# at-cg/PHI

Hardware: AMD Instinct MI355X
Metric: read Gbases/s scored (49-hap MHC graph stand-in synMHC-49); reads resident in HBM, parsing and H2D excluded (higher is better)
Workload: dtype u64

## Files before the change

phi_amd/build.py:

```python
import os
import subprocess
import sys

ROOT = os.path.dirname(os.path.dirname(os.path.abspath(__file__)))
CSRC = os.path.join(ROOT, "phi_amd", "csrc")
HIPCC = os.environ.get("HIPCC", "/opt/rocm/bin/hipcc")
ARCH = "gfx950"

HIP_SOURCES = ["sketch.hip", "sketch_pooled.hip", "sketch_win_fixed.hip", "table.hip", "anchors.hip", "contexts.hip", "dp.hip", "dp_events.hip", "dp_blocks.hip", "phi_abi.hip", "dev_mem.hip", "read_batches.hip", "text_stream.hip", "text_park.hip", "set_graph.hip", "phi_solve.hip", "solve_dev.hip", "phi_comm.hip", "phi_ipc.hip", "reads_text.hip", "walk_text.hip", "edit.hip", "edit_path.hip", "inflate.hip", "gfa_text.hip", "chop.hip", "vcf.hip", "ladder.hip", "panel.hip", "panel_score.hip", "scan.hip", "bam.hip", "calls.hip", "deflate.hip"]
HIP_HEADERS = ["phi_dev.h", "phi_kernels.h", "phi_ctx.h", "phi_dp_flags.h", "phi_host_par.h", "phi_wave.h", "dp_dev.h", "dp_steps.h", "solve_host.h", "reads_host.h", "bam_header.h", "deflate_codes.h", "sketch_dev.h", "sketch_phases.inc", "sketch_minima.inc", "sketch_rounds.inc", "sketch_rounds_kmer.inc", "edit_band.inc", os.path.join("host", "panel_choose.h"), os.path.join("..", "..", "include", "phi_amd.h")]


def _run(cmd, cwd=None):
    print("+", " ".join(cmd), flush=True)
    subprocess.check_call(cmd, cwd=cwd)


def _stale(target, deps):
    if not os.path.exists(target):
        return True
    t = os.path.getmtime(target)
    return any(os.path.getmtime(d) > t for d in deps if os.path.exists(d))


EXTRA_FLAGS = {"sketch_pooled.hip": ["-mllvm", "-disable-machine-licm"]}


def build_device(force=False):
    objdir = os.path.join(ROOT, "build", "obj")
    os.makedirs(objdir, exist_ok=True)
    hdrs = [os.path.join(CSRC, h) for h in HIP_HEADERS]
    objs = []
    for src in HIP_SOURCES:
        s = os.path.join(CSRC, src)
        o = os.path.join(objdir, src.replace(".hip", ".o"))
        if force or _stale(o, [s] + hdrs):
            _run([HIPCC, f"--offload-arch={ARCH}", "-O3", "-std=c++17", "-fPIC", "-Wall", "-Wno-unused-function"]
                 + EXTRA_FLAGS.get(src, []) + ["-c", s, "-o", o])
        objs.append(o)
    lib = os.path.join(ROOT, "phi_amd", "libphi_amd.so")
    if force or _stale(lib, objs):
        tmp = f"{lib}.{os.getpid()}.tmp"
        _run([HIPCC, f"--offload-arch={ARCH}", "-shared", "-fPIC", "-o", tmp] + objs + ["-ldl"])
        os.replace(tmp, lib)
    return lib


def build_host(force=False):
    hostdir = os.path.join(CSRC, "host")
    if not os.path.isdir(hostdir):
        return None
    _run(["make", "-C", hostdir] + (["-B"] if force else []))
    return os.path.join(ROOT, "phi_amd", "libphi_host.so")


def build_all(force=False):
    build_device(force)
    build_host(force)


if __name__ == "__main__":
    build_all(force="--force" in sys.argv)
```

phi_amd/csrc/dp_events.hip:

```cpp
#include <hip/hip_runtime.h>
#include "phi_kernels.h"
#include "dp_dev.h"

#define CHK PHI_DP_CHUNK
#define RING PHI_DP_RING
enum { DP_SEQ = 0, DP_ROW = 1, DP_PATH = 2 };

__global__ void __launch_bounds__(256) phi_event_flags_kernel(const int32_t *__restrict__ walk_vtx, int64_t n_entries,
                                                              const int32_t *__restrict__ cvtx, uint8_t *__restrict__ flags)
{
    for (int64_t e = (int64_t)blockIdx.x * blockDim.x + threadIdx.x; e < n_entries; e += (int64_t)gridDim.x * blockDim.x)
        flags[e] = cvtx[walk_vtx[e]] >= 0;
}

__global__ void phi_event_off_kernel(const phi_ent_t *__restrict__ ev_e, int64_t n_ev, const int64_t *__restrict__ walk_off,
                                     int32_t n_walks, int64_t *__restrict__ ev_off)
{
    const int h = blockIdx.x * blockDim.x + threadIdx.x;
    if (h > n_walks) return;
    const int64_t key = walk_off[h];
    int64_t lo = 0, hi = n_ev;
    while (lo < hi) {
        const int64_t mid = (lo + hi) >> 1;
        if ((int64_t)ev_e[mid] < key) lo = mid + 1; else hi = mid;
// ... 167 lines not shown
    const int h = threadIdx.x;
    const bool has_walk = h < A.n_walks;
    const int64_t eb = has_walk ? A.walk_off[h] : 0;
    const int64_t ee = has_walk ? A.walk_off[h + 1] : 0;
    const int32_t sb = MODE == DP_PATH ? (int32_t)blockIdx.x : 0;
    const int32_t kbeg = MODE == DP_PATH ? A.blk_lo[sb] : 0, kend = MODE == DP_PATH ? A.blk_lo[sb + 1] : A.n_k;
    const int64_t vb = !has_walk ? 0 : MODE == DP_PATH ? (int64_t)A.blk_ev[(int64_t)sb * A.lane_stride + h] : A.ev_off[h];
    const int64_t ve = has_walk ? A.ev_off[h + 1] : 0;
    int64_t vi = vb;
    int64_t wl = vb;
    const uint4 *evg = reinterpret_cast<const uint4 *>(A.ev);

    uint4 wtmp[P][3];
    int64_t whi = vb;
    auto issue = [&]() {
        whi = min(ve, vi + D);
#pragma unroll
        for (int j = 0; j < P; j++) {
            const int64_t x = (ve > vb) ? min(wl + j, ve - 1) : 0;
            wtmp[j][0] = evg[x * 3 + 0]; wtmp[j][1] = evg[x * 3 + 1]; wtmp[j][2] = evg[x * 3 + 2];
        }
    };
    auto land = [&]() {
#pragma unroll
        for (int j = 0; j < P; j++) {
            const int64_t x = wl + j;
            if (x < whi) {
                const int sl = (int)(x & (D - 1));
                s_ev[sl][0][h] = wtmp[j][0]; s_ev[sl][1][h] = wtmp[j][1]; s_ev[sl][2][h] = wtmp[j][2];
            }
        }
        wl = max(wl, min(whi, wl + P));
    };
    if (A.n_ev > 0) { issue(); land(); issue(); land(); }
    uint4 cA = make_uint4(0xFFFFFFFFu, 0, 0, 0);
    if (vi < ve) cA = s_ev[vi & (D - 1)][0][h];

    int32_t qh = 0, qt = 0;
    int32_t M = NEGK, sL = 0, Emax = NEG;
    if (MODE == DP_PATH) { sL = -1; if (has_walk) M = A.blk_S[(int64_t)sb * A.lane_stride + h]; }

    const int32_t n_steps = kend - kbeg;
    const int n_chunks = (n_steps + CHK - 1) / CHK;
    auto stage = [&](int c) {
        const int b = c & 1;
        const int32_t s0 = kbeg + c * CHK;
        const int32_t ns = min(CHK, kend - s0);
        const int4 *src = reinterpret_cast<const int4 *>(A.k_rec + (int64_t)s0 * 8);
        int4 *dst = &s_rec[b][0][0];
        for (int i = h; i < ns * 2; i += NT) dst[i] = src[i];
    };
    stage(0);
    __syncthreads();

    for (int c = 0; c < n_chunks; c++) {
        const int b = c & 1;
        if (c + 1 < n_chunks) stage(c + 1);
        const int32_t s0 = kbeg + c * CHK;
        const int32_t ns = min(CHK, kend - s0);
        int4 ra = s_rec[b][0][0], rb = s_rec[b][0][1];
        for (int i = 0; i < ns; i++) {
            const int inx = min(i + 1, CHK - 1);
            const int4 na = s_rec[b][inx][0], nb = s_rec[b][inx][1];
            if ((c | i) && (i & (P - 1)) == 0) issue();
            if ((c | i) && (i & (P - 1)) == P / 2) {
                land();
                if (vi < ve) cA = s_ev[vi & (D - 1)][0][h];
            }
            const int32_t k = s0 + i;
            const int32_t flags = ra.x;
            const bool active = (int32_t)(cA.x & 0x7FFFFFFFu) == k;

            int32_t E = NEG, Eh = -1, Esrc = -1;
            if (flags & PHI_DP_NEED_ENTRY) {
                dp_eval_entry<RNG, true>(ra, rb, k, s_top, A.k_in_packed, reinterpret_cast<const int4 *>(A.tops), A.cost, E, Eh, Esrc);
                if (h == 0) { A.ent_src[k] = Esrc; A.ent_h[k] = Eh; }
            }

            int32_t dmax = NEG;
            int32_t oidx = 255;
            if (active) {
                const int64_t e = (int64_t)cA.y;
                const bool ovf = (cA.x >> 31) != 0;
                const int32_t t = (int32_t)(e - eb);
                const int32_t End = (int32_t)cA.z, SB = (int32_t)cA.w;
                const int sl = (int)(vi & (D - 1));
                const uint8_t *gb = reinterpret_cast<const uint8_t *>(&s_ev[sl][1][h]);
                oidx = reinterpret_cast<const uint8_t *>(&s_ev[sl][2][h])[15];
                while (qh != qt && t - s_qs[qh & (QD - 1)][h] >= 31) {
                    const int32_t key = s_qK[qh & (QD - 1)][h];
                    if (key > M) { M = key; sL = s_qs[qh & (QD - 1)][h]; }
                    qh++;
                }
                int32_t newE = NEG;
                if (t == 0) { newE = 0; qh = qt = 0; M = NEGK; Emax = NEG; }
                else if ((flags & PHI_DP_NEED_ENTRY) && Eh >= 0) newE = E;
                if (newE > Emax) {
                    Emax = newE;
                    const int32_t key = newE - SB;
                    while (qh != qt && s_qK[(qt - 1) & (QD - 1)][h] < key) qt--;
                    if (qt - qh >= q_limit) { atomicOr(A.err, PHI_KERR_DP_QUEUE); qt--; }
                    s_qs[qt & (QD - 1)][h] = t; s_qE[qt & (QD - 1)][h] = newE; s_qK[qt & (QD - 1)][h] = key;
                    qt++;
                }
                if ((flags & PHI_DP_NEED_TOPS) || e == ee - 1) {
                    int32_t best = M > NEGK / 2 ? M + End : NEG, bs = sL;
                    for (int32_t j = qh; j != qt; j++) {
                        const int32_t s = s_qs[j & (QD - 1)][h];
                        const int a = t - s;
                        int32_t inside;
                        if (!ovf) inside = a < 16 ? gb[a] : reinterpret_cast<const uint8_t *>(&s_ev[sl][2][h])[a - 16];
                        else inside = ev_count_inside(A, eb + s, e);
                        const int32_t val = s_qE[j & (QD - 1)][h] + inside;
                        if (val > best) { best = val; bs = s; }
                    }
                    if (best > NEG / 2) { dmax = best; A.dmax[e] = best; A.bstart[e] = bs; }
                    else { A.dmax[e] = NEG; A.bstart[e] = 0; }
                }
                vi++;
                cA = make_uint4(0xFFFFFFFFu, 0, 0, 0);
                if (vi < ve) cA = s_ev[vi & (D - 1)][0][h];
            }

            if (flags & PHI_DP_NEED_TOPS) {
                const bool leaving = active && oidx != 255 && dmax > NEG / 2;
                const DpTops t = dp_tops_waves<NW>(leaving, dmax, oidx, s_red, s_oidx);
                if (h == 0) {
                    const int4 q = pack_tops(t);
                    s_top[k & (RNG - 1)] = q;
                    reinterpret_cast<int4 *>(A.tops)[k] = q;
                }
                __syncthreads();
            }
            ra = na; rb = nb;
        }
        __threadfence_block();
        __syncthreads();
    }
    if (MODE == DP_PATH) {
        int32_t best = M > NEGK / 2 ? M : NEGK, bs = sL;
        for (int32_t j = qh; j != qt; j++) {
            const int32_t key = s_qK[j & (QD - 1)][h];
            if (key > best) { best = key; bs = s_qs[j & (QD - 1)][h]; }
        }
        A.blk_keys_out[(int64_t)sb * A.lane_stride + h] = (has_walk && vb < ve) ? best : NEGK;
        A.blk_carry[(int64_t)sb * A.lane_stride + h] = bs;
    }
}


template <int NPW, int MODE, int P, int RINGT, int QD, int CK = CHK>
__global__ void __launch_bounds__(64 * (1 + NPW)) phi_dp_events_pc_kernel(PhiDpEventArgs A)
{
    constexpr int D = 2 * P;
    constexpr int PER_CHUNK = CK / P;
    static_assert(P % NPW == 0 && CK % P == 0, "ring geometry");
    __shared__ int4 s_rec[2 * CK][2];
    __shared__ int4 s_top[RINGT];
    __shared__ int2 s_ent[2 * P];
    __shared__ uint4 s_ev[D][3][64];
    __shared__ int4 s_res[D][64];
    __shared__ int32_t s_qs[QD][64], s_qE[QD][64], s_qK[QD][64];
    __shared__ int32_t s_vi[2][64];

    const int wave = threadIdx.x >> 6, h = threadIdx.x & 63;
    const bool cls = MODE == DP_ROW && A.lane_walk != nullptr;
    const unsigned n_rows = cls ? 65u : (unsigned)(A.n_walks + 1);
    int32_t sb = 0, row_j = -1;
    if (MODE == DP_ROW) { sb = (int32_t)(blockIdx.x / n_rows); row_j = (int32_t)(blockIdx.x % n_rows); }
    if (MODE == DP_PATH) sb = (int32_t)blockIdx.x;
    const bool start_row = MODE == DP_ROW && row_j == (int32_t)n_rows - 1;
    int32_t w = h;
    bool has_walk = h < A.n_walks;
    if (cls) { w = A.lane_walk[(int64_t)sb * 64 + h]; has_walk = w >= 0; if (!has_walk) w = 0; }
    const int32_t k0 = MODE == DP_SEQ ? 0 : A.blk_lo[sb];
    const int32_t k1 = MODE == DP_SEQ ? A.n_k : A.blk_lo[sb + 1];
    const int32_t n_steps = k1 - k0;
    const phi_ent_t eb = has_walk ? (phi_ent_t)A.walk_off[w] : 0;
    const phi_ent_t e_last = has_walk ? (phi_ent_t)(A.walk_off[w + 1] - 1) : 0xFFFFFFFFu;
    const int32_t v0 = has_walk ? (int32_t)A.ev_off[w] : 0;
    const int32_t ve = has_walk ? (int32_t)A.ev_off[w + 1] : 0;
    const int32_t vb = MODE == DP_SEQ ? v0 : (has_walk ? A.blk_ev[(int64_t)sb * A.lane_stride + w] : 0);
    const int n_per = (n_steps + P - 1) / P;
    if (MODE == DP_ROW && !start_row) {
        const int32_t wj = cls ? A.lane_walk[(int64_t)sb * 64 + row_j] : row_j;
        if (wj < 0) return;
        const int32_t jb = A.blk_ev[(int64_t)sb * A.lane_stride + wj];
        if (jb <= (int32_t)A.ev_off[wj] || jb >= (int32_t)A.ev_off[wj + 1]) {
            if (wave == 0) {
                A.row_out[(int64_t)blockIdx.x * 64 + h] = NEGK;
                if (h == 0) { A.rowend_out[blockIdx.x] = NEG; if (A.rownew_out) A.rownew_out[blockIdx.x] = NEGK; if (A.rowdiag_out) A.rowdiag_out[(int64_t)sb * 64 + row_j] = NEGK; }
            }
            return;
        }
    }

    if (wave > 0) {
        const int pw = wave - 1;
        const uint4 *evg = reinterpret_cast<const uint4 *>(A.ev);
        auto stage = [&](int c) {
            const int32_t s0 = k0 + c * CK;
            const int32_t ns = min(CK, k1 - s0);
            const int4 *src = reinterpret_cast<const int4 *>(A.k_rec + (int64_t)s0 * 8);
            int4 *dst = &s_rec[(c & 1) * CK][0];
            for (int i = pw * 64 + h; i < ns * 2; i += 64 * NPW) dst[i] = src[i];
        };
        stage(0);
#pragma unroll
        for (int n = 0; n < D / NPW; n++) {
            const int32_t x = vb + pw + n * NPW;
            if (x < ve) {
                const uint4 a = evg[(int64_t)x * 3 + 0], g0 = evg[(int64_t)x * 3 + 1], g1 = evg[(int64_t)x * 3 + 2];
                s_ev[x & (D - 1)][0][h] = a; s_ev[x & (D - 1)][1][h] = g0; s_ev[x & (D - 1)][2][h] = g1;
            }
        }
        int32_t wl = min(ve, vb + D);
        int32_t vprev = vb;
        __syncthreads();
        for (int p = 0;; p++) {
            const int32_t vi = has_walk ? s_vi[p & 1][h] : 0;
            if (MODE != DP_ROW) {
#pragma unroll
                for (int n = 0; n < P / NPW; n++) {
                    const int32_t x = vprev + pw + n * NPW;
                    if (x < vi) {
                        const int4 r = s_res[x & (D - 1)][h];
                        A.dmax[(phi_ent_t)r.z] = r.x; A.bstart[(phi_ent_t)r.z] = r.y;
                    }
                }
                if (pw == 0 && p > 0 && h < P) {
                    const int32_t r = (p - 1) * P + h;
                    if (r < n_steps) {
                        const int32_t k = k0 + r;
                        reinterpret_cast<int4 *>(A.tops)[k] = s_top[k & (RINGT - 1)];
                        const int2 en = s_ent[r & (2 * P - 1)];
                        A.ent_src[k] = en.x; A.ent_h[k] = en.y;
                    }
                }
            }
            if (p == n_per) break;
            const int32_t hi = min(ve, vi + D);
            uint4 t0[P / NPW], t1[P / NPW], t2[P / NPW];
#pragma unroll
            for (int n = 0; n < P / NPW; n++) {
                const int64_t xc = (ve > v0) ? min(wl + pw + n * NPW, ve - 1) : 0;
                t0[n] = evg[xc * 3 + 0]; t1[n] = evg[xc * 3 + 1]; t2[n] = evg[xc * 3 + 2];
            }
#pragma unroll
            for (int n = 0; n < P / NPW; n++) {
                const int32_t x = wl + pw + n * NPW;
                if (x < hi) { s_ev[x & (D - 1)][0][h] = t0[n]; s_ev[x & (D - 1)][1][h] = t1[n]; s_ev[x & (D - 1)][2][h] = t2[n]; }
            }
            wl = max(wl, min(hi, wl + P));
            if (p % PER_CHUNK == 0 && (p / PER_CHUNK + 1) * CK < n_steps) stage(p / PER_CHUNK + 1);
            vprev = vi;
            __syncthreads();
        }
        return;
    }

    int32_t vi = vb;
    s_vi[0][h] = vi;
    __syncthreads();
    uint4 cA = make_uint4(0xFFFFFFFFu, 0, 0, 0);
    if (vi < ve) cA = s_ev[vi & (D - 1)][0][h];
    int32_t qh = 0, qn = 0, hs = 0, hE = 0, tk = 0;
    int32_t M = NEGK, sL = MODE == DP_SEQ ? 0 : -1, Emax = NEG;
    if (MODE == DP_ROW && h == row_j) M = 0;
    if (MODE == DP_PATH && has_walk) M = A.blk_S[(int64_t)sb * A.lane_stride + h];
    const bool starts_on = MODE != DP_ROW || start_row;
    int32_t endbest = NEG;
    int32_t Kn = NEGK;
    int4 ra = s_rec[0][0], rb = s_rec[0][1];
    int4 lastq = make_int4(NEG, NEG, 0, 0);
    int32_t lastk = -1;

    auto eval_entry = [&](const int4 xa, const int4 xb, int32_t k, int32_t &E, int32_t &Eh, int32_t &Esrc) {
        const uint32_t b0 = (uint32_t)xa.z >> 8;
        if (((xa.x >> 8) & 0xFF) == 1 && b0 < RINGT) {
            const int32_t src = k - (int32_t)b0;
            int32_t val, hh;
            tops_for_edge(src == lastk ? lastq : s_top[src & (RINGT - 1)], xa.z & 0xFF, val, hh);
            E = NEG; Eh = -1; Esrc = -1;
            if (hh >= 0) { E = val - A.cost; Eh = hh; Esrc = src; }
        } else {
            dp_eval_entry<RINGT, MODE != DP_ROW>(xa, xb, k, s_top, A.k_in_packed, reinterpret_cast<const int4 *>(A.tops), A.cost, E, Eh, Esrc);
        }
        if (h == 0) s_ent[(k - k0) & (2 * P - 1)] = make_int2(Esrc, Eh);
    };

    for (int p = 0; p < n_per; p++) {
        const int32_t r_end = min(n_steps, (p + 1) * P);
        if (vi < ve) cA = s_ev[vi & (D - 1)][0][h];
        for (int32_t r = p * P; r < r_end;) {
            const int32_t k = k0 + r;
            const int4 na = s_rec[(r + 1) & (2 * CK - 1)][0], nb = s_rec[(r + 1) & (2 * CK - 1)][1];
            const int4 n2a = s_rec[(r + 2) & (2 * CK - 1)][0], n2b = s_rec[(r + 2) & (2 * CK - 1)][1];
            const bool pair = (ra.x & PHI_DP_PAIR) && r + 1 < r_end;
            const int32_t stepk = (int32_t)(cA.x & 0x7FFFFFFFu);
            const bool second = pair && stepk == k + 1;
            const bool active = stepk == k || second;
            const int32_t flags = second ? na.x : ra.x;

            int32_t E = NEG, Eh = -1, Esrc = -1;
            if (ra.x & PHI_DP_NEED_ENTRY) eval_entry(ra, rb, k, E, Eh, Esrc);
            if (pair && (na.x & PHI_DP_NEED_ENTRY)) {
                int32_t E1, Eh1, Esrc1;
                eval_entry(na, nb, k + 1, E1, Eh1, Esrc1);
                if (second) { E = E1; Eh = Eh1; Esrc = Esrc1; }
            } else if (second) { E = NEG; Eh = -1; }

            int32_t dmax = NEG;
            int32_t oidx = 255;
            if (active) {
                const int sl = (int)(vi & (D - 1));
                const phi_ent_t e = cA.y;
                const bool ovf = (cA.x >> 31) != 0;
                const int32_t t = (int32_t)(e - eb);
                const int32_t End = (int32_t)cA.z, SB = (int32_t)cA.w;
                const uint8_t *gb = reinterpret_cast<const uint8_t *>(&s_ev[sl][1][h]);
                oidx = gb[15 + 1024];
                while (qn > 0 && t - hs >= 31) {
                    const int32_t key = qn == 1 ? tk : s_qK[qh & (QD - 1)][h];
                    if (key > M) { M = key; sL = hs; }
                    qh++; qn--;
                    if (qn > 0) { hs = s_qs[qh & (QD - 1)][h]; hE = s_qE[qh & (QD - 1)][h]; }
                }
                int32_t newE = NEG;
                if (t == 0) { newE = starts_on ? 0 : NEG; qn = 0; M = NEGK; Emax = NEG; }
                else if ((flags & PHI_DP_NEED_ENTRY) && Eh >= 0) newE = E;
                if (newE > Emax) {
                    Emax = newE;
                    const int32_t key = newE - SB;
                    while (qn > 0 && tk < key) {
                        qn--;
                        if (qn > 0) tk = s_qK[(qh + qn - 1) & (QD - 1)][h];
                    }
                    if (QD < 32 && qn == QD) { atomicOr(A.err, PHI_KERR_DP_QUEUE); qn--; }
                    const int slq = (qh + qn) & (QD - 1);
                    s_qs[slq][h] = t; s_qE[slq][h] = newE; s_qK[slq][h] = key;
                    if (qn == 0) { hs = t; hE = newE; }
                    tk = key;
                    qn++;
                    if (MODE == DP_ROW && key > Kn) Kn = key;
                }
                int32_t bs = 0;
                if ((flags & PHI_DP_NEED_TOPS) || e == e_last) {
                    int32_t best = M > NEGK / 2 ? M + End : NEG;
                    bs = sL;
                    for (int32_t j = 0; j < qn; j++) {
                        const int32_t s = j == 0 ? hs : s_qs[(qh + j) & (QD - 1)][h];
                        const int32_t Es = j == 0 ? hE : s_qE[(qh + j) & (QD - 1)][h];
                        const int a = t - s;
                        const int32_t inside = !ovf ? (int32_t)gb[(a & 15) + (a >> 4) * 1024] : ev_count_inside(A, (int64_t)eb + s, e);
                        const int32_t val = Es + inside;
                        if (val > best) { best = val; bs = s; }
                    }
                    if (best > NEG / 2) dmax = best; else bs = 0;
                    if (MODE == DP_ROW && e == e_last) endbest = max(endbest, dmax);
                }
                s_res[sl][h] = make_int4(dmax, bs, (int32_t)e, 0);
                vi++;
                cA = make_uint4(0xFFFFFFFFu, 0, 0, 0);
                if (vi < ve) cA = s_ev[vi & (D - 1)][0][h];
            }

            if (!pair && (ra.x & PHI_DP_NEED_TOPS)) {
                const bool leaving = active && oidx != 255 && dmax > NEG / 2;
                DpTops t;
                if (__ballot(leaving && oidx > 1) == 0ull) {
                    const bool on0 = leaving && oidx == 0, on1 = leaving && oidx == 1;
                    unsigned long long K0, K1;
                    ev_wave_max2_key(on0 ? ev_key(dmax, h) : 0ull, on1 ? ev_key(dmax, h) : 0ull, K0, K1);
                    const bool first0 = K0 >= K1;
                    const unsigned long long Kf = first0 ? K0 : K1, Ks = first0 ? K1 : K0;
                    t.t1v = Kf ? (int32_t)(uint32_t)(Kf >> 8) + NEG : NEG;
                    t.t1h = Kf ? 255 - (int32_t)(Kf & 255) : -1;
                    t.t1n = Kf ? (first0 ? 0 : 1) : -1;
                    t.t2v = Ks ? (int32_t)(uint32_t)(Ks >> 8) + NEG : NEG;
                    t.t2h = Ks ? 255 - (int32_t)(Ks & 255) : -1;
                } else {
                    t = dp_tops_wave(leaving, dmax, oidx);
                }
                lastq = pack_tops(t);
                lastk = k;
                if (h == 0) s_top[k & (RINGT - 1)] = lastq;
            }
            if (pair) { ra = n2a; rb = n2b; r += 2; }
            else { ra = na; rb = nb; r += 1; }
        }
        s_vi[(p + 1) & 1][h] = vi;
        __syncthreads();
    }
    if (MODE != DP_SEQ) {
        int32_t best = M > NEGK / 2 ? M : NEGK, bs = sL;
        for (int32_t j = 0; j < qn; j++) {
            const int32_t key = s_qK[(qh + j) & (QD - 1)][h];
            if (key > best) { best = key; bs = s_qs[(qh + j) & (QD - 1)][h]; }
        }
        if (MODE == DP_ROW) {
            const bool on_diag = A.rowdiag_out && h == row_j;
            if (on_diag) A.rowdiag_out[(int64_t)sb * 64 + h] = has_walk ? best : NEGK;
            A.row_out[(int64_t)blockIdx.x * 64 + h] = has_walk && !on_diag ? best : NEGK;
            const int32_t eb_all = wave_max_i32(endbest);
            if (h == 0) A.rowend_out[blockIdx.x] = eb_all;
            if (A.rownew_out && h == row_j) A.rownew_out[blockIdx.x] = Kn;
            if (A.rownew_out && start_row && h == 0) A.rownew_out[blockIdx.x] = NEGK;
        } else {
            A.blk_keys_out[(int64_t)sb * A.lane_stride + h] = (has_walk && vb < ve) ? best : NEGK;
            A.blk_carry[(int64_t)sb * A.lane_stride + h] = bs;
        }
    }
}

void phi_launch_dp_block_paths_wide(hipStream_t st, const PhiDpEventArgs &A)
{
    if (A.n_walks <= 128) hipLaunchKernelGGL((phi_dp_events_kernel<2, DP_PATH>), dim3((unsigned)A.n_blk), dim3(128), 0, st, A);
    else hipLaunchKernelGGL((phi_dp_events_kernel<4, DP_PATH>), dim3((unsigned)A.n_blk), dim3(256), 0, st, A);
}

void phi_launch_dp_events(hipStream_t st, const PhiDpEventArgs &A)
{
    if (A.n_walks <= 64) hipLaunchKernelGGL((phi_dp_events_pc_kernel<2, DP_SEQ, 8, RING, 32>), dim3(1), dim3(64 * 3), 0, st, A);
    else if (A.n_walks <= 128) hipLaunchKernelGGL((phi_dp_events_kernel<2, DP_SEQ>), dim3(1), dim3(128), 0, st, A);
    else hipLaunchKernelGGL((phi_dp_events_kernel<4, DP_SEQ>), dim3(1), dim3(256), 0, st, A);
}

void phi_launch_dp_block_rows(hipStream_t st, const PhiDpEventArgs &A)
{
    const unsigned grid = (unsigned)A.n_blk * (A.lane_walk ? 65u : (unsigned)(A.n_walks + 1));
    if (A.blk_ring <= 256 && A.blk_max_len > 0 && A.blk_max_len <= 64 && !getenv("PHI_DP_ROWS_LARGE"))
        hipLaunchKernelGGL((phi_dp_events_pc_kernel<2, DP_ROW, 2, 64, 8, 32>), dim3(grid), dim3(64 * 3), 0, st, A);
    else if (A.blk_ring <= 256) hipLaunchKernelGGL((phi_dp_events_pc_kernel<2, DP_ROW, 2, 256, 8>), dim3(grid), dim3(64 * 3), 0, st, A);
    else if (A.blk_ring <= 1024) hipLaunchKernelGGL((phi_dp_events_pc_kernel<2, DP_ROW, 4, 1024, 16>), dim3(grid), dim3(64 * 3), 0, st, A);
    else hipLaunchKernelGGL((phi_dp_events_pc_kernel<2, DP_ROW, 4, 2048, 16>), dim3(grid), dim3(64 * 3), 0, st, A);
}
void phi_launch_dp_block_paths(hipStream_t st, const PhiDpEventArgs &A)
{
    if (A.blk_ring <= 256) hipLaunchKernelGGL((phi_dp_events_pc_kernel<2, DP_PATH, 4, 256, 8>), dim3((unsigned)A.n_blk), dim3(64 * 3), 0, st, A);
    else if (A.blk_ring <= 1024) hipLaunchKernelGGL((phi_dp_events_pc_kernel<2, DP_PATH, 4, 1024, 16>), dim3((unsigned)A.n_blk), dim3(64 * 3), 0, st, A);
    else hipLaunchKernelGGL((phi_dp_events_pc_kernel<2, DP_PATH, 4, 2048, 16>), dim3((unsigned)A.n_blk), dim3(64 * 3), 0, st, A);
}

__global__ void phi_warm_dp_events_kernel() {}
void phi_warm_dp_events(hipStream_t st) { hipLaunchKernelGGL(phi_warm_dp_events_kernel, dim3(1), dim3(64), 0, st); }
```

Measured before the change: 473.8.

## Group multiple DP row computations per block sharing one producer-staged event buffer

Moves the producer/consumer DP kernel body into a shared include and adds a grouped row kernel in which NC compute waves, each handling a different row of the same block, share one set of producer waves that stage events and records into LDS. This amortises global loads and staging across rows and cuts the number of launched blocks. It also skips the s_res writes in row mode, which row mode never reads. Group size defaults to 2 for small blocks and 13 otherwise, with an environment override, at the cost of larger workgroups and more shared-memory pressure.

After: 472.6 (median of 2 runs). About the same (-0.2%).

```diff
diff --git a/phi_amd/build.py b/phi_amd/build.py
--- a/phi_amd/build.py
+++ b/phi_amd/build.py
@@ -8,7 +8,7 @@
 ARCH = "gfx950"
 
 HIP_SOURCES = ["sketch.hip", "sketch_pooled.hip", "sketch_win_fixed.hip", "table.hip", "anchors.hip", "contexts.hip", "dp.hip", "dp_events.hip", "dp_blocks.hip", "phi_abi.hip", "dev_mem.hip", "read_batches.hip", "text_stream.hip", "text_park.hip", "set_graph.hip", "phi_solve.hip", "solve_dev.hip", "phi_comm.hip", "phi_ipc.hip", "reads_text.hip", "walk_text.hip", "edit.hip", "edit_path.hip", "inflate.hip", "gfa_text.hip", "chop.hip", "vcf.hip", "ladder.hip", "panel.hip", "panel_score.hip", "scan.hip", "bam.hip", "calls.hip", "deflate.hip"]
-HIP_HEADERS = ["phi_dev.h", "phi_kernels.h", "phi_ctx.h", "phi_dp_flags.h", "phi_host_par.h", "phi_wave.h", "dp_dev.h", "dp_steps.h", "solve_host.h", "reads_host.h", "bam_header.h", "deflate_codes.h", "sketch_dev.h", "sketch_phases.inc", "sketch_minima.inc", "sketch_rounds.inc", "sketch_rounds_kmer.inc", "edit_band.inc", os.path.join("host", "panel_choose.h"), os.path.join("..", "..", "include", "phi_amd.h")]
+HIP_HEADERS = ["phi_dev.h", "phi_kernels.h", "phi_ctx.h", "phi_dp_flags.h", "phi_host_par.h", "phi_wave.h", "dp_dev.h", "dp_events_pc.inc", "dp_steps.h", "solve_host.h", "reads_host.h", "bam_header.h", "deflate_codes.h", "sketch_dev.h", "sketch_phases.inc", "sketch_minima.inc", "sketch_rounds.inc", "sketch_rounds_kmer.inc", "edit_band.inc", os.path.join("host", "panel_choose.h"), os.path.join("..", "..", "include", "phi_amd.h")]
 
 
 def _run(cmd, cwd=None):
diff --git a/phi_amd/csrc/dp_events.hip b/phi_amd/csrc/dp_events.hip
--- a/phi_amd/csrc/dp_events.hip
+++ b/phi_amd/csrc/dp_events.hip
@@ -343,265 +343,14 @@
 template <int NPW, int MODE, int P, int RINGT, int QD, int CK = CHK>
 __global__ void __launch_bounds__(64 * (1 + NPW)) phi_dp_events_pc_kernel(PhiDpEventArgs A)
 {
-    constexpr int D = 2 * P;
-    constexpr int PER_CHUNK = CK / P;
-    static_assert(P % NPW == 0 && CK % P == 0, "ring geometry");
-    __shared__ int4 s_rec[2 * CK][2];
-    __shared__ int4 s_top[RINGT];
-    __shared__ int2 s_ent[2 * P];
-    __shared__ uint4 s_ev[D][3][64];
-    __shared__ int4 s_res[D][64];
-    __shared__ int32_t s_qs[QD][64], s_qE[QD][64], s_qK[QD][64];
-    __shared__ int32_t s_vi[2][64];
-
-    const int wave = threadIdx.x >> 6, h = threadIdx.x & 63;
-    const bool cls = MODE == DP_ROW && A.lane_walk != nullptr;
-    const unsigned n_rows = cls ? 65u : (unsigned)(A.n_walks + 1);
-    int32_t sb = 0, row_j = -1;
-    if (MODE == DP_ROW) { sb = (int32_t)(blockIdx.x / n_rows); row_j = (int32_t)(blockIdx.x % n_rows); }
-    if (MODE == DP_PATH) sb = (int32_t)blockIdx.x;
-    const bool start_row = MODE == DP_ROW && row_j == (int32_t)n_rows - 1;
-    int32_t w = h;
-    bool has_walk = h < A.n_walks;
-    if (cls) { w = A.lane_walk[(int64_t)sb * 64 + h]; has_walk = w >= 0; if (!has_walk) w = 0; }
-    const int32_t k0 = MODE == DP_SEQ ? 0 : A.blk_lo[sb];
-    const int32_t k1 = MODE == DP_SEQ ? A.n_k : A.blk_lo[sb + 1];
-    const int32_t n_steps = k1 - k0;
-    const phi_ent_t eb = has_walk ? (phi_ent_t)A.walk_off[w] : 0;
-    const phi_ent_t e_last = has_walk ? (phi_ent_t)(A.walk_off[w + 1] - 1) : 0xFFFFFFFFu;
-    const int32_t v0 = has_walk ? (int32_t)A.ev_off[w] : 0;
-    const int32_t ve = has_walk ? (int32_t)A.ev_off[w + 1] : 0;
-    const int32_t vb = MODE == DP_SEQ ? v0 : (has_walk ? A.blk_ev[(int64_t)sb * A.lane_stride + w] : 0);
-    const int n_per = (n_steps + P - 1) / P;
-    if (MODE == DP_ROW && !start_row) {
-        const int32_t wj = cls ? A.lane_walk[(int64_t)sb * 64 + row_j] : row_j;
-        if (wj < 0) return;
-        const int32_t jb = A.blk_ev[(int64_t)sb * A.lane_stride + wj];
-        if (jb <= (int32_t)A.ev_off[wj] || jb >= (int32_t)A.ev_off[wj + 1]) {
-            if (wave == 0) {
-                A.row_out[(int64_t)blockIdx.x * 64 + h] = NEGK;
-                if (h == 0) { A.rowend_out[blockIdx.x] = NEG; if (A.rownew_out) A.rownew_out[blockIdx.x] = NEGK; if (A.rowdiag_out) A.rowdiag_out[(int64_t)sb * 64 + row_j] = NEGK; }
-            }
-            return;
-        }
-    }
-
-    if (wave > 0) {
-        const int pw = wave - 1;
-        const uint4 *evg = reinterpret_cast<const uint4 *>(A.ev);
-        auto stage = [&](int c) {
-            const int32_t s0 = k0 + c * CK;
-            const int32_t ns = min(CK, k1 - s0);
-            const int4 *src = reinterpret_cast<const int4 *>(A.k_rec + (int64_t)s0 * 8);
-            int4 *dst = &s_rec[(c & 1) * CK][0];
-            for (int i = pw * 64 + h; i < ns * 2; i += 64 * NPW) dst[i] = src[i];
-        };
-        stage(0);
-#pragma unroll
-        for (int n = 0; n < D / NPW; n++) {
-            const int32_t x = vb + pw + n * NPW;
-            if (x < ve) {
-                const uint4 a = evg[(int64_t)x * 3 + 0], g0 = evg[(int64_t)x * 3 + 1], g1 = evg[(int64_t)x * 3 + 2];
-                s_ev[x & (D - 1)][0][h] = a; s_ev[x & (D - 1)][1][h] = g0; s_ev[x & (D - 1)][2][h] = g1;
-            }
-        }
-        int32_t wl = min(ve, vb + D);
-        int32_t vprev = vb;
-        __syncthreads();
-        for (int p = 0;; p++) {
-            const int32_t vi = has_walk ? s_vi[p & 1][h] : 0;
-            if (MODE != DP_ROW) {
-#pragma unroll
-                for (int n = 0; n < P / NPW; n++) {
-                    const int32_t x = vprev + pw + n * NPW;
-                    if (x < vi) {
-                        const int4 r = s_res[x & (D - 1)][h];
-                        A.dmax[(phi_ent_t)r.z] = r.x; A.bstart[(phi_ent_t)r.z] = r.y;
-                    }
-                }
-                if (pw == 0 && p > 0 && h < P) {
-                    const int32_t r = (p - 1) * P + h;
-                    if (r < n_steps) {
-                        const int32_t k = k0 + r;
-                        reinterpret_cast<int4 *>(A.tops)[k] = s_top[k & (RINGT - 1)];
-                        const int2 en = s_ent[r & (2 * P - 1)];
-                        A.ent_src[k] = en.x; A.ent_h[k] = en.y;
-                    }
-                }
-            }
-            if (p == n_per) break;
-            const int32_t hi = min(ve, vi + D);
-            uint4 t0[P / NPW], t1[P / NPW], t2[P / NPW];
-#pragma unroll
-            for (int n = 0; n < P / NPW; n++) {
-                const int64_t xc = (ve > v0) ? min(wl + pw + n * NPW, ve - 1) : 0;
-                t0[n] = evg[xc * 3 + 0]; t1[n] = evg[xc * 3 + 1]; t2[n] = evg[xc * 3 + 2];
-            }
-#pragma unroll
-            for (int n = 0; n < P / NPW; n++) {
-                const int32_t x = wl + pw + n * NPW;
-                if (x < hi) { s_ev[x & (D - 1)][0][h] = t0[n]; s_ev[x & (D - 1)][1][h] = t1[n]; s_ev[x & (D - 1)][2][h] = t2[n]; }
-            }
-            wl = max(wl, min(hi, wl + P));
-            if (p % PER_CHUNK == 0 && (p / PER_CHUNK + 1) * CK < n_steps) stage(p / PER_CHUNK + 1);
-            vprev = vi;
-            __syncthreads();
-        }
-        return;
-    }
-
-    int32_t vi = vb;
-    s_vi[0][h] = vi;
-    __syncthreads();
-    uint4 cA = make_uint4(0xFFFFFFFFu, 0, 0, 0);
-    if (vi < ve) cA = s_ev[vi & (D - 1)][0][h];
-    int32_t qh = 0, qn = 0, hs = 0, hE = 0, tk = 0;
-    int32_t M = NEGK, sL = MODE == DP_SEQ ? 0 : -1, Emax = NEG;
-    if (MODE == DP_ROW && h == row_j) M = 0;
-    if (MODE == DP_PATH && has_walk) M = A.blk_S[(int64_t)sb * A.lane_stride + h];
-    const bool starts_on = MODE != DP_ROW || start_row;
-    int32_t endbest = NEG;
-    int32_t Kn = NEGK;
-    int4 ra = s_rec[0][0], rb = s_rec[0][1];
-    int4 lastq = make_int4(NEG, NEG, 0, 0);
-    int32_t lastk = -1;
-
-    auto eval_entry = [&](const int4 xa, const int4 xb, int32_t k, int32_t &E, int32_t &Eh, int32_t &Esrc) {
-        const uint32_t b0 = (uint32_t)xa.z >> 8;
-        if (((xa.x >> 8) & 0xFF) == 1 && b0 < RINGT) {
-            const int32_t src = k - (int32_t)b0;
-            int32_t val, hh;
-            tops_for_edge(src == lastk ? lastq : s_top[src & (RINGT - 1)], xa.z & 0xFF, val, hh);
-            E = NEG; Eh = -1; Esrc = -1;
-            if (hh >= 0) { E = val - A.cost; Eh = hh; Esrc = src; }
-        } else {
-            dp_eval_entry<RINGT, MODE != DP_ROW>(xa, xb, k, s_top, A.k_in_packed, reinterpret_cast<const int4 *>(A.tops), A.cost, E, Eh, Esrc);
-        }
-        if (h == 0) s_ent[(k - k0) & (2 * P - 1)] = make_int2(Esrc, Eh);
-    };
-
-    for (int p = 0; p < n_per; p++) {
-        const int32_t r_end = min(n_steps, (p + 1) * P);
-        if (vi < ve) cA = s_ev[vi & (D - 1)][0][h];
-        for (int32_t r = p * P; r < r_end;) {
-            const int32_t k = k0 + r;
-            const int4 na = s_rec[(r + 1) & (2 * CK - 1)][0], nb = s_rec[(r + 1) & (2 * CK - 1)][1];
-            const int4 n2a = s_rec[(r + 2) & (2 * CK - 1)][0], n2b = s_rec[(r + 2) & (2 * CK - 1)][1];
-            const bool pair = (ra.x & PHI_DP_PAIR) && r + 1 < r_end;
-            const int32_t stepk = (int32_t)(cA.x & 0x7FFFFFFFu);
-            const bool second = pair && stepk == k + 1;
-            const bool active = stepk == k || second;
-            const int32_t flags = second ? na.x : ra.x;
-
-            int32_t E = NEG, Eh = -1, Esrc = -1;
-            if (ra.x & PHI_DP_NEED_ENTRY) eval_entry(ra, rb, k, E, Eh, Esrc);
-            if (pair && (na.x & PHI_DP_NEED_ENTRY)) {
-                int32_t E1, Eh1, Esrc1;
-                eval_entry(na, nb, k + 1, E1, Eh1, Esrc1);
-                if (second) { E = E1; Eh = Eh1; Esrc = Esrc1; }
-            } else if (second) { E = NEG; Eh = -1; }
-
-            int32_t dmax = NEG;
-            int32_t oidx = 255;
-            if (active) {
-                const int sl = (int)(vi & (D - 1));
-                const phi_ent_t e = cA.y;
-                const bool ovf = (cA.x >> 31) != 0;
-                const int32_t t = (int32_t)(e - eb);
-                const int32_t End = (int32_t)cA.z, SB = (int32_t)cA.w;
-                const uint8_t *gb = reinterpret_cast<const uint8_t *>(&s_ev[sl][1][h]);
-                oidx = gb[15 + 1024];
-                while (qn > 0 && t - hs >= 31) {
-                    const int32_t key = qn == 1 ? tk : s_qK[qh & (QD - 1)][h];
-                    if (key > M) { M = key; sL = hs; }
-                    qh++; qn--;
-                    if (qn > 0) { hs = s_qs[qh & (QD - 1)][h]; hE = s_qE[qh & (QD - 1)][h]; }
-                }
-                int32_t newE = NEG;
-                if (t == 0) { newE = starts_on ? 0 : NEG; qn = 0; M = NEGK; Emax = NEG; }
-                else if ((flags & PHI_DP_NEED_ENTRY) && Eh >= 0) newE = E;
-                if (newE > Emax) {
-                    Emax = newE;
-                    const int32_t key = newE - SB;
-                    while (qn > 0 && tk < key) {
-                        qn--;
-                        if (qn > 0) tk = s_qK[(qh + qn - 1) & (QD - 1)][h];
-                    }
-                    if (QD < 32 && qn == QD) { atomicOr(A.err, PHI_KERR_DP_QUEUE); qn--; }
-                    const int slq = (qh + qn) & (QD - 1);
-                    s_qs[slq][h] = t; s_qE[slq][h] = newE; s_qK[slq][h] = key;
-                    if (qn == 0) { hs = t; hE = newE; }
-                    tk = key;
-                    qn++;
-                    if (MODE == DP_ROW && key > Kn) Kn = key;
-                }
-                int32_t bs = 0;
-                if ((flags & PHI_DP_NEED_TOPS) || e == e_last) {
-                    int32_t best = M > NEGK / 2 ? M + End : NEG;
-                    bs = sL;
-                    for (int32_t j = 0; j < qn; j++) {
-                        const int32_t s = j == 0 ? hs : s_qs[(qh + j) & (QD - 1)][h];
-                        const int32_t Es = j == 0 ? hE : s_qE[(qh + j) & (QD - 1)][h];
-                        const int a = t - s;
-                        const int32_t inside = !ovf ? (int32_t)gb[(a & 15) + (a >> 4) * 1024] : ev_count_inside(A, (int64_t)eb + s, e);
-                        const int32_t val = Es + inside;
-                        if (val > best) { best = val; bs = s; }
-                    }
-                    if (best > NEG / 2) dmax = best; else bs = 0;
-                    if (MODE == DP_ROW && e == e_last) endbest = max(endbest, dmax);
-                }
-                s_res[sl][h] = make_int4(dmax, bs, (int32_t)e, 0);
-                vi++;
-                cA = make_uint4(0xFFFFFFFFu, 0, 0, 0);
-                if (vi < ve) cA = s_ev[vi & (D - 1)][0][h];
-            }
-
-            if (!pair && (ra.x & PHI_DP_NEED_TOPS)) {
-                const bool leaving = active && oidx != 255 && dmax > NEG / 2;
-                DpTops t;
-                if (__ballot(leaving && oidx > 1) == 0ull) {
-                    const bool on0 = leaving && oidx == 0, on1 = leaving && oidx == 1;
-                    unsigned long long K0, K1;
-                    ev_wave_max2_key(on0 ? ev_key(dmax, h) : 0ull, on1 ? ev_key(dmax, h) : 0ull, K0, K1);
-                    const bool first0 = K0 >= K1;
-                    const unsigned long long Kf = first0 ? K0 : K1, Ks = first0 ? K1 : K0;
-                    t.t1v = Kf ? (int32_t)(uint32_t)(Kf >> 8) + NEG : NEG;
-                    t.t1h = Kf ? 255 - (int32_t)(Kf & 255) : -1;
-                    t.t1n = Kf ? (first0 ? 0 : 1) : -1;
-                    t.t2v = Ks ? (int32_t)(uint32_t)(Ks >> 8) + NEG : NEG;
-                    t.t2h = Ks ? 255 - (int32_t)(Ks & 255) : -1;
-                } else {
-                    t = dp_tops_wave(leaving, dmax, oidx);
-                }
-                lastq = pack_tops(t);
-                lastk = k;
-                if (h == 0) s_top[k & (RINGT - 1)] = lastq;
-            }
-            if (pair) { ra = n2a; rb = n2b; r += 2; }
-            else { ra = na; rb = nb; r += 1; }
-        }
-        s_vi[(p + 1) & 1][h] = vi;
-        __syncthreads();
-    }
-    if (MODE != DP_SEQ) {
-        int32_t best = M > NEGK / 2 ? M : NEGK, bs = sL;
-        for (int32_t j = 0; j < qn; j++) {
-            const int32_t key = s_qK[(qh + j) & (QD - 1)][h];
-            if (key > best) { best = key; bs = s_qs[(qh + j) & (QD - 1)][h]; }
-        }
-        if (MODE == DP_ROW) {
-            const bool on_diag = A.rowdiag_out && h == row_j;
-            if (on_diag) A.rowdiag_out[(int64_t)sb * 64 + h] = has_walk ? best : NEGK;
-            A.row_out[(int64_t)blockIdx.x * 64 + h] = has_walk && !on_diag ? best : NEGK;
-            const int32_t eb_all = wave_max_i32(endbest);
-            if (h == 0) A.rowend_out[blockIdx.x] = eb_all;
-            if (A.rownew_out && h == row_j) A.rownew_out[blockIdx.x] = Kn;
-            if (A.rownew_out && start_row && h == 0) A.rownew_out[blockIdx.x] = NEGK;
-        } else {
-            A.blk_keys_out[(int64_t)sb * A.lane_stride + h] = (has_walk && vb < ve) ? best : NEGK;
-            A.blk_carry[(int64_t)sb * A.lane_stride + h] = bs;
-        }
-    }
+    constexpr int NC = 1;
+#include "dp_events_pc.inc"
+}
+template <int NC, int P, int RINGT, int QD, int CK>
+__global__ void __launch_bounds__(64 * (NC + 2)) phi_dp_rows_group_kernel(PhiDpEventArgs A)
+{
+    constexpr int NPW = 2, MODE = DP_ROW;
+#include "dp_events_pc.inc"
 }
 
 void phi_launch_dp_block_paths_wide(hipStream_t st, const PhiDpEventArgs &A)
@@ -617,11 +366,39 @@
     else hipLaunchKernelGGL((phi_dp_events_kernel<4, DP_SEQ>), dim3(1), dim3(256), 0, st, A);
 }
 
+#define PHI_DP_ROW_GROUPS(X) X(2) X(4) X(5) X(6) X(8) X(13)
+template <int P, int RINGT, int QD, int CK>
+static void dp_launch_row_groups(hipStream_t st, const PhiDpEventArgs &A, unsigned n_rows, int nc)
+{
+    const unsigned grid = (unsigned)A.n_blk * ((n_rows + (unsigned)nc - 1) / (unsigned)nc);
+    switch (nc) {
+#define X(N) case N: hipLaunchKernelGGL((phi_dp_rows_group_kernel<N, P, RINGT, QD, CK>), dim3(grid), dim3(64 * (N + 2)), 0, st, A); break;
+    PHI_DP_ROW_GROUPS(X)
+#undef X
+    default: break;
+    }
+}
+static int dp_row_group(int want)
+{
+    int nc = 1;
+#define X(N) if (N <= want) nc = N;
+    PHI_DP_ROW_GROUPS(X)
+#undef X
+    return nc;
+}
 void phi_launch_dp_block_rows(hipStream_t st, const PhiDpEventArgs &A)
 {
-    const unsigned grid = (unsigned)A.n_blk * (A.lane_walk ? 65u : (unsigned)(A.n_walks + 1));
-    if (A.blk_ring <= 256 && A.blk_max_len > 0 && A.blk_max_len <= 64 && !getenv("PHI_DP_ROWS_LARGE"))
-        hipLaunchKernelGGL((phi_dp_events_pc_kernel<2, DP_ROW, 2, 64, 8, 32>), dim3(grid), dim3(64 * 3), 0, st, A);
+    const unsigned n_rows = A.lane_walk ? 65u : (unsigned)(A.n_walks + 1);
+    const unsigned grid = (unsigned)A.n_blk * n_rows;
+    const bool small = A.blk_ring <= 256 && A.blk_max_len > 0 && A.blk_max_len <= 64 && !getenv("PHI_DP_ROWS_LARGE");
+    const char *force = getenv("PHI_DP_ROW_GROUP");
+    int nc = A.blk_ring > 256 ? 1 : small ? 2 : 13;
+    if (force && atoi(force) >= 1) nc = A.blk_ring > 256 ? 1 : dp_row_group(atoi(force));
+    if (nc > 1) {
+        if (small) dp_launch_row_groups<2, 64, 8, 32>(st, A, n_rows, nc);
+        else dp_launch_row_groups<2, 256, 8, CHK>(st, A, n_rows, nc);
+    }
+    else if (small) hipLaunchKernelGGL((phi_dp_events_pc_kernel<2, DP_ROW, 2, 64, 8, 32>), dim3(grid), dim3(64 * 3), 0, st, A);
     else if (A.blk_ring <= 256) hipLaunchKernelGGL((phi_dp_events_pc_kernel<2, DP_ROW, 2, 256, 8>), dim3(grid), dim3(64 * 3), 0, st, A);
     else if (A.blk_ring <= 1024) hipLaunchKernelGGL((phi_dp_events_pc_kernel<2, DP_ROW, 4, 1024, 16>), dim3(grid), dim3(64 * 3), 0, st, A);
     else hipLaunchKernelGGL((phi_dp_events_pc_kernel<2, DP_ROW, 4, 2048, 16>), dim3(grid), dim3(64 * 3), 0, st, A);
diff --git a/phi_amd/csrc/dp_events_pc.inc b/phi_amd/csrc/dp_events_pc.inc
--- /dev/null
+++ b/phi_amd/csrc/dp_events_pc.inc
@@ -0,0 +1,286 @@
+    constexpr int D = 2 * P;
+    constexpr int PER_CHUNK = CK / P;
+    static_assert(P % NPW == 0 && CK % P == 0, "ring geometry");
+    static_assert(NC == 1 || MODE == DP_ROW, "only the rows are grouped");
+    __shared__ int4 s_rec[2 * CK][2];
+    __shared__ int4 s_top_c[NC][RINGT];
+    __shared__ int2 s_ent_c[NC][2 * P];
+    __shared__ uint4 s_ev[D][3][64];
+    __shared__ int4 s_res[MODE == DP_ROW ? 1 : D][64];
+    __shared__ int32_t s_qs_c[NC][QD][64], s_qE_c[NC][QD][64], s_qK_c[NC][QD][64];
+    __shared__ int32_t s_vi[2][64];
+
+    const int wave = threadIdx.x >> 6, h = threadIdx.x & 63;
+    const int cw = NC == 1 || wave >= NC ? 0 : wave;
+    auto &s_top = s_top_c[cw];
+    auto &s_ent = s_ent_c[cw];
+    auto &s_qs = s_qs_c[cw];
+    auto &s_qE = s_qE_c[cw];
+    auto &s_qK = s_qK_c[cw];
+    const bool cls = MODE == DP_ROW && A.lane_walk != nullptr;
+    const unsigned n_rows = cls ? 65u : (unsigned)(A.n_walks + 1);
+    const unsigned n_grp = (n_rows + NC - 1) / NC;
+    int32_t sb = 0, row_j = -1, grp = 0;
+    if (MODE == DP_ROW) { sb = (int32_t)(blockIdx.x / n_grp); grp = (int32_t)(blockIdx.x % n_grp); row_j = grp * NC + cw; }
+    if (MODE == DP_PATH) sb = (int32_t)blockIdx.x;
+    const bool start_row = MODE == DP_ROW && row_j == (int32_t)n_rows - 1;
+    const int64_t orow = (int64_t)sb * n_rows + row_j;
+    int32_t w = h;
+    bool has_walk = h < A.n_walks;
+    if (cls) { w = A.lane_walk[(int64_t)sb * 64 + h]; has_walk = w >= 0; if (!has_walk) w = 0; }
+    const int32_t k0 = MODE == DP_SEQ ? 0 : A.blk_lo[sb];
+    const int32_t k1 = MODE == DP_SEQ ? A.n_k : A.blk_lo[sb + 1];
+    const int32_t n_steps = k1 - k0;
+    const phi_ent_t eb = has_walk ? (phi_ent_t)A.walk_off[w] : 0;
+    const phi_ent_t e_last = has_walk ? (phi_ent_t)(A.walk_off[w + 1] - 1) : 0xFFFFFFFFu;
+    const int32_t v0 = has_walk ? (int32_t)A.ev_off[w] : 0;
+    const int32_t ve = has_walk ? (int32_t)A.ev_off[w + 1] : 0;
+    const int32_t vb = MODE == DP_SEQ ? v0 : (has_walk ? A.blk_ev[(int64_t)sb * A.lane_stride + w] : 0);
+    const int n_per = (n_steps + P - 1) / P;
+    int lead = 0;
+    if (MODE == DP_ROW) {
+        unsigned live = 0;
+#pragma unroll
+        for (int c = 0; c < NC; c++) {
+            const int32_t rj = grp * NC + c;
+            if (rj >= (int32_t)n_rows) continue;
+            if (rj == (int32_t)n_rows - 1) { live |= 1u << c; continue; }
+            const int32_t wj = cls ? A.lane_walk[(int64_t)sb * 64 + rj] : rj;
+            if (wj < 0) continue;
+            const int32_t jb = A.blk_ev[(int64_t)sb * A.lane_stride + wj];
+            if (jb <= (int32_t)A.ev_off[wj] || jb >= (int32_t)A.ev_off[wj + 1]) {
+                if (wave == c) {
+                    A.row_out[orow * 64 + h] = NEGK;
+                    if (h == 0) { A.rowend_out[orow] = NEG; if (A.rownew_out) A.rownew_out[orow] = NEGK; if (A.rowdiag_out) A.rowdiag_out[(int64_t)sb * 64 + row_j] = NEGK; }
+                }
+                continue;
+            }
+            live |= 1u << c;
+        }
+        if (live == 0) return;
+        lead = __builtin_ctz(live);
+        if (NC > 1 && wave < NC && !((live >> wave) & 1u)) {
+            for (int p = 0; p <= n_per; p++) __syncthreads();
+            return;
+        }
+    }
+
+    if (wave >= NC) {
+        const int pw = wave - NC;
+        const uint4 *evg = reinterpret_cast<const uint4 *>(A.ev);
+        auto stage = [&](int c) {
+            const int32_t s0 = k0 + c * CK;
+            const int32_t ns = min(CK, k1 - s0);
+            const int4 *src = reinterpret_cast<const int4 *>(A.k_rec + (int64_t)s0 * 8);
+            int4 *dst = &s_rec[(c & 1) * CK][0];
+            for (int i = pw * 64 + h; i < ns * 2; i += 64 * NPW) dst[i] = src[i];
+        };
+        stage(0);
+#pragma unroll
+        for (int n = 0; n < D / NPW; n++) {
+            const int32_t x = vb + pw + n * NPW;
+            if (x < ve) {
+                const uint4 a = evg[(int64_t)x * 3 + 0], g0 = evg[(int64_t)x * 3 + 1], g1 = evg[(int64_t)x * 3 + 2];
+                s_ev[x & (D - 1)][0][h] = a; s_ev[x & (D - 1)][1][h] = g0; s_ev[x & (D - 1)][2][h] = g1;
+            }
+        }
+        int32_t wl = min(ve, vb + D);
+        int32_t vprev = vb;
+        __syncthreads();
+        for (int p = 0;; p++) {
+            const int32_t vi = has_walk ? s_vi[p & 1][h] : 0;
+            if (MODE != DP_ROW) {
+#pragma unroll
+                for (int n = 0; n < P / NPW; n++) {
+                    const int32_t x = vprev + pw + n * NPW;
+                    if (x < vi) {
+                        const int4 r = s_res[x & (D - 1)][h];
+                        A.dmax[(phi_ent_t)r.z] = r.x; A.bstart[(phi_ent_t)r.z] = r.y;
+                    }
+                }
+                if (pw == 0 && p > 0 && h < P) {
+                    const int32_t r = (p - 1) * P + h;
+                    if (r < n_steps) {
+                        const int32_t k = k0 + r;
+                        reinterpret_cast<int4 *>(A.tops)[k] = s_top[k & (RINGT - 1)];
+                        const int2 en = s_ent[r & (2 * P - 1)];
+                        A.ent_src[k] = en.x; A.ent_h[k] = en.y;
+                    }
+                }
+            }
+            if (p == n_per) break;
+            const int32_t hi = min(ve, vi + D);
+            uint4 t0[P / NPW], t1[P / NPW], t2[P / NPW];
+#pragma unroll
+            for (int n = 0; n < P / NPW; n++) {
+                const int64_t xc = (ve > v0) ? min(wl + pw + n * NPW, ve - 1) : 0;
+                t0[n] = evg[xc * 3 + 0]; t1[n] = evg[xc * 3 + 1]; t2[n] = evg[xc * 3 + 2];
+            }
+#pragma unroll
+            for (int n = 0; n < P / NPW; n++) {
+                const int32_t x = wl + pw + n * NPW;
+                if (x < hi) { s_ev[x & (D - 1)][0][h] = t0[n]; s_ev[x & (D - 1)][1][h] = t1[n]; s_ev[x & (D - 1)][2][h] = t2[n]; }
+            }
+            wl = max(wl, min(hi, wl + P));
+            if (p % PER_CHUNK == 0 && (p / PER_CHUNK + 1) * CK < n_steps) stage(p / PER_CHUNK + 1);
+            vprev = vi;
+            __syncthreads();
+        }
+        return;
+    }
+
+    int32_t vi = vb;
+    if (NC == 1 || cw == lead) s_vi[0][h] = vi;
+    __syncthreads();
+    uint4 cA = make_uint4(0xFFFFFFFFu, 0, 0, 0);
+    if (vi < ve) cA = s_ev[vi & (D - 1)][0][h];
+    int32_t qh = 0, qn = 0, hs = 0, hE = 0, tk = 0;
+    int32_t M = NEGK, sL = MODE == DP_SEQ ? 0 : -1, Emax = NEG;
+    if (MODE == DP_ROW && h == row_j) M = 0;
+    if (MODE == DP_PATH && has_walk) M = A.blk_S[(int64_t)sb * A.lane_stride + h];
+    const bool starts_on = MODE != DP_ROW || start_row;
+    int32_t endbest = NEG;
+    int32_t Kn = NEGK;
+    int4 ra = s_rec[0][0], rb = s_rec[0][1];
+    int4 lastq = make_int4(NEG, NEG, 0, 0);
+    int32_t lastk = -1;
+
+    auto eval_entry = [&](const int4 xa, const int4 xb, int32_t k, int32_t &E, int32_t &Eh, int32_t &Esrc) {
+        const uint32_t b0 = (uint32_t)xa.z >> 8;
+        if (((xa.x >> 8) & 0xFF) == 1 && b0 < RINGT) {
+            const int32_t src = k - (int32_t)b0;
+            int32_t val, hh;
+            tops_for_edge(src == lastk ? lastq : s_top[src & (RINGT - 1)], xa.z & 0xFF, val, hh);
+            E = NEG; Eh = -1; Esrc = -1;
+            if (hh >= 0) { E = val - A.cost; Eh = hh; Esrc = src; }
+        } else {
+            dp_eval_entry<RINGT, MODE != DP_ROW>(xa, xb, k, s_top, A.k_in_packed, reinterpret_cast<const int4 *>(A.tops), A.cost, E, Eh, Esrc);
+        }
+        if (h == 0) s_ent[(k - k0) & (2 * P - 1)] = make_int2(Esrc, Eh);
+    };
+
+    for (int p = 0; p < n_per; p++) {
+        const int32_t r_end = min(n_steps, (p + 1) * P);
+        if (vi < ve) cA = s_ev[vi & (D - 1)][0][h];
+        for (int32_t r = p * P; r < r_end;) {
+            const int32_t k = k0 + r;
+            const int4 na = s_rec[(r + 1) & (2 * CK - 1)][0], nb = s_rec[(r + 1) & (2 * CK - 1)][1];
+            const int4 n2a = s_rec[(r + 2) & (2 * CK - 1)][0], n2b = s_rec[(r + 2) & (2 * CK - 1)][1];
+            const bool pair = (ra.x & PHI_DP_PAIR) && r + 1 < r_end;
+            const int32_t stepk = (int32_t)(cA.x & 0x7FFFFFFFu);
+            const bool second = pair && stepk == k + 1;
+            const bool active = stepk == k || second;
+            const int32_t flags = second ? na.x : ra.x;
+
+            int32_t E = NEG, Eh = -1, Esrc = -1;
+            if (ra.x & PHI_DP_NEED_ENTRY) eval_entry(ra, rb, k, E, Eh, Esrc);
+            if (pair && (na.x & PHI_DP_NEED_ENTRY)) {
+                int32_t E1, Eh1, Esrc1;
+                eval_entry(na, nb, k + 1, E1, Eh1, Esrc1);
+                if (second) { E = E1; Eh = Eh1; Esrc = Esrc1; }
+            } else if (second) { E = NEG; Eh = -1; }
+
+            int32_t dmax = NEG;
+            int32_t oidx = 255;
+            if (active) {
+                const int sl = (int)(vi & (D - 1));
+                const phi_ent_t e = cA.y;
+                const bool ovf = (cA.x >> 31) != 0;
+                const int32_t t = (int32_t)(e - eb);
+                const int32_t End = (int32_t)cA.z, SB = (int32_t)cA.w;
+                const uint8_t *gb = reinterpret_cast<const uint8_t *>(&s_ev[sl][1][h]);
+                oidx = gb[15 + 1024];
+                while (qn > 0 && t - hs >= 31) {
+                    const int32_t key = qn == 1 ? tk : s_qK[qh & (QD - 1)][h];
+                    if (key > M) { M = key; sL = hs; }
+                    qh++; qn--;
+                    if (qn > 0) { hs = s_qs[qh & (QD - 1)][h]; hE = s_qE[qh & (QD - 1)][h]; }
+                }
+                int32_t newE = NEG;
+                if (t == 0) { newE = starts_on ? 0 : NEG; qn = 0; M = NEGK; Emax = NEG; }
+                else if ((flags & PHI_DP_NEED_ENTRY) && Eh >= 0) newE = E;
+                if (newE > Emax) {
+                    Emax = newE;
+                    const int32_t key = newE - SB;
+                    while (qn > 0 && tk < key) {
+                        qn--;
+                        if (qn > 0) tk = s_qK[(qh + qn - 1) & (QD - 1)][h];
+                    }
+                    if (QD < 32 && qn == QD) { atomicOr(A.err, PHI_KERR_DP_QUEUE); qn--; }
+                    const int slq = (qh + qn) & (QD - 1);
+                    s_qs[slq][h] = t; s_qE[slq][h] = newE; s_qK[slq][h] = key;
+                    if (qn == 0) { hs = t; hE = newE; }
+                    tk = key;
+                    qn++;
+                    if (MODE == DP_ROW && key > Kn) Kn = key;
+                }
+                int32_t bs = 0;
+                if ((flags & PHI_DP_NEED_TOPS) || e == e_last) {
+                    int32_t best = M > NEGK / 2 ? M + End : NEG;
+                    bs = sL;
+                    for (int32_t j = 0; j < qn; j++) {
+                        const int32_t s = j == 0 ? hs : s_qs[(qh + j) & (QD - 1)][h];
+                        const int32_t Es = j == 0 ? hE : s_qE[(qh + j) & (QD - 1)][h];
+                        const int a = t - s;
+                        const int32_t inside = !ovf ? (int32_t)gb[(a & 15) + (a >> 4) * 1024] : ev_count_inside(A, (int64_t)eb + s, e);
+                        const int32_t val = Es + inside;
+                        if (val > best) { best = val; bs = s; }
+                    }
+                    if (best > NEG / 2) dmax = best; else bs = 0;
+                    if (MODE == DP_ROW && e == e_last) endbest = max(endbest, dmax);
+                }
+                if (MODE != DP_ROW) s_res[sl][h] = make_int4(dmax, bs, (int32_t)e, 0);
+                vi++;
+                cA = make_uint4(0xFFFFFFFFu, 0, 0, 0);
+                if (vi < ve) cA = s_ev[vi & (D - 1)][0][h];
+            }
+
+            if (!pair && (ra.x & PHI_DP_NEED_TOPS)) {
+                const bool leaving = active && oidx != 255 && dmax > NEG / 2;
+                DpTops t;
+                if (__ballot(leaving && oidx > 1) == 0ull) {
+                    const bool on0 = leaving && oidx == 0, on1 = leaving && oidx == 1;
+                    unsigned long long K0, K1;
+                    ev_wave_max2_key(on0 ? ev_key(dmax, h) : 0ull, on1 ? ev_key(dmax, h) : 0ull, K0, K1);
+                    const bool first0 = K0 >= K1;
+                    const unsigned long long Kf = first0 ? K0 : K1, Ks = first0 ? K1 : K0;
+                    t.t1v = Kf ? (int32_t)(uint32_t)(Kf >> 8) + NEG : NEG;
+                    t.t1h = Kf ? 255 - (int32_t)(Kf & 255) : -1;
+                    t.t1n = Kf ? (first0 ? 0 : 1) : -1;
+                    t.t2v = Ks ? (int32_t)(uint32_t)(Ks >> 8) + NEG : NEG;
+                    t.t2h = Ks ? 255 - (int32_t)(Ks & 255) : -1;
+                } else {
+                    t = dp_tops_wave(leaving, dmax, oidx);
+                }
+                lastq = pack_tops(t);
+                lastk = k;
+                if (h == 0) s_top[k & (RINGT - 1)] = lastq;
+            }
+            if (pair) { ra = n2a; rb = n2b; r += 2; }
+            else { ra = na; rb = nb; r += 1; }
+        }
+        if (NC == 1 || cw == lead) s_vi[(p + 1) & 1][h] = vi;
+        __syncthreads();
+#ifdef PHI_DP_GROUP_CHECK
+        if (NC > 1 && cw != lead && has_walk && s_vi[(p + 1) & 1][h] != vi) atomicOr(A.err, PHI_KERR_DP_QUEUE);
+#endif
+    }
+    if (MODE != DP_SEQ) {
+        int32_t best = M > NEGK / 2 ? M : NEGK, bs = sL;
+        for (int32_t j = 0; j < qn; j++) {
+            const int32_t key = s_qK[(qh + j) & (QD - 1)][h];
+            if (key > best) { best = key; bs = s_qs[(qh + j) & (QD - 1)][h]; }
+        }
+        if (MODE == DP_ROW) {
+            const bool on_diag = A.rowdiag_out && h == row_j;
+            if (on_diag) A.rowdiag_out[(int64_t)sb * 64 + h] = has_walk ? best : NEGK;
+            A.row_out[orow * 64 + h] = has_walk && !on_diag ? best : NEGK;
+            const int32_t eb_all = wave_max_i32(endbest);
+            if (h == 0) A.rowend_out[orow] = eb_all;
+            if (A.rownew_out && h == row_j) A.rownew_out[orow] = Kn;
+            if (A.rownew_out && start_row && h == 0) A.rownew_out[orow] = NEGK;
+        } else {
+            A.blk_keys_out[(int64_t)sb * A.lane_stride + h] = (has_walk && vb < ve) ? best : NEGK;
+            A.blk_carry[(int64_t)sb * A.lane_stride + h] = bs;
+        }
+    }
```
